# feifeibear/long-context-attention

Hardware: AMD Instinct MI355X
Metric: attention TFLOP/s (algorithmic, causal fwd+bwd) + iter ms of LongContextAttention at seqlen 64K, ulysses x ring (higher is better)
Workload: dtype bf16

## Files before the change

### long-context-attention_amd/csrc/usp_flash_bwd_dq64.hip

```cpp
#ifdef USP_Q64_TIMING
#define USP_TIMING
#endif
#include "usp_bwd_params.hpp"
#include "usp_host.hpp"
#include "usp_mfma64.hpp"

namespace usp {

#ifndef USP_Q64_PF
#define USP_Q64_PF 3
#endif
constexpr int kQ64_PF = USP_Q64_PF;
#ifndef USP_Q64_Y1
#define USP_Q64_Y1 24
#endif
constexpr int kQ64_Y1 = USP_Q64_Y1;

template <int DT, bool CAUSAL>
__global__ __launch_bounds__(256, 1) void flash_bwd_dq64_kernel(const BwdParams ) {
  using E = Elem<DT>;
  using M = M64<DT>;
  constexpr int D = 128, kBM = 256;
  constexpr int ROWB = D * 2;
  constexpr int TILEB = kTile * ROWB;
  constexpr int VOFF = 2 * TILEB;
  constexpr int NKT = D / 16, NDJ = D / 32;
  constexpr int PF = kQ64_PF;

  extern __shared__ __attribute__((aligned(16))) char smem_raw[];
  USP_LDS char* smem = lds_block_at_zero(smem_raw);

  const int tid = threadIdx.x;
  const int lane = tid & 63;
  const int wave = __builtin_amdgcn_readfirstlane(tid >> 6);
  const int l31 = lane & 31;
  const int hi = lane >> 5;
  typedef const __attribute__((address_space(4))) BwdParams* KArgs;
  KArgs p = (KArgs)__builtin_amdgcn_kernarg_segment_ptr();
  asm volatile("" : "+s"(p));

  const int dma_row = lane >> 4, dma_c8 = dma_lane_col(lane & 15, dma_row);
  const int k_voff = dma_row * (int)p->k_ss * 2 + dma_c8, v_voff = dma_row * (int)p->v_ss * 2 + dma_c8;
  const int rd_base = l31 * ROWB + ((hi ^ tile_swz<D>(l31)) * 16);
  int tr_addr[NDJ][2];
  {
    const int i = lane & 15, grp = (lane >> 4) & 1;
#pragma unroll
    for (int dj = 0; dj < NDJ; ++dj)
#pragma unroll
      for (int e = 0; e < 2; ++e) tr_addr[dj][e] = tr_read_offset<D>(i, grp, hi, dj, e);
  }
  const float c = p->scale_log2;

  const ItemWalk walk(p->n_items);
  for (int pass = 0;; ++pass) {
  int w = walk.at(pass);
  if (w < 0) break;
  asm volatile("" : "+s"(p));
  USP_TM(const uint64_t tm_item = __builtin_amdgcn_s_memtime();)
  w = walk.dealt(w, p->nblk);
  if (p->ksplit <= 1) w = walk.grouped(w, p->nblk, p->walk_g);
  const int qt_r = w % p->nblk;
  int rest = w / p->nblk;
  const int qt = CAUSAL ? (p->nblk - 1 - qt_r) : qt_r;
  int cut = 0;
  if (p->ksplit > 1) { cut = rest % p->ksplit; rest /= p->ksplit; }
  const int h = rest % p->Hq, b = rest / p->Hq;
  const int hkv = h / p->G;
  const int q0 = qt * kBM;
  const int qw = q0 + wave * 64;
  const int off = p->causal_off;

  const usp_query_tiles kr = usp_query_tiles_of(q0, kBM, qw, 64, p->Sq, p->Sk, CAUSAL, off, kTile);
  const int nt = kr.nt, n_w = kr.n_w, n_full = kr.n_full;
  usp_tile_run run = {0, nt};
  if (p->ksplit > 1) run = usp_equal_run(0, nt, p->ksplit, cut);
  const int tb = run.begin, te = run.end;
  const int e_full = usp_clamp_to_run(n_full, tb, te);
  const int e_own = usp_clamp_to_run(n_w, tb, te);

  u32x4 qf[2][NKT], df[2][NKT];
  float nl[2], dl[2];
#pragma unroll
  for (int qb = 0; qb < 2; ++qb) {
    const int row = qw + 32 * qb + l31;
    const int row_c = row < p->Sq ? row : p->Sq - 1;
    const char* qp = p->q + 2 * (b * p->q_sb + (int64_t)row_c * p->q_ss + h * p->q_sh) + 16 * hi;
    const char* dp = p->dout + 2 * (b * p->do_sb + (int64_t)row_c * p->do_ss + h * p->do_sh) + 16 * hi;
    load_resident16(qf[qb], df[qb], qp, dp);
    const float lse = p->lse[b * p->lse_sb + h * p->lse_sh + row_c];
    const float dlt = p->delta[b * p->dl_sb + h * p->dl_sh + row_c];
    const bool live = row < p->Sq && lse != USP_NEG_INF;
    nl[qb] = live ? -lse * kLog2e : USP_NEG_INF;
    dl[qb] = live ? dlt : 0.f;
  }

  const int k_rowb = (int)p->k_ss * 2, v_rowb = (int)p->v_ss * 2;
  const int64_t k_tb = (int64_t)kTile * k_rowb, v_tb = (int64_t)kTile * v_rowb;
  int k_step = 4 * k_rowb - 1024, v_step = 4 * v_rowb - 1024;
  int lds_w = wave * 4096;
  const char* k_cur = p->k + 2 * (b * p->k_sb + hkv * p->k_sh) + (int64_t)wave * 16 * k_rowb + tb * k_tb;
  const char* v_cur = p->v + 2 * (b * p->v_sb + hkv * p->v_sh) + (int64_t)wave * 16 * v_rowb + tb * v_tb;
  int rows_kv = p->Sk - 16 * wave - tb * kTile;
  u32x4 k_rs, v_rs;
  int dma_buf = 0;
  auto dma_open = [&](int buf) {
    k_rs = make_rsrc_rows(k_cur, rows_kv, 16, k_rowb, 2 * D);
    v_rs = make_rsrc_rows(v_cur, rows_kv, 16, v_rowb, 2 * D);
    dma_buf = buf;
    k_cur += k_tb;
    v_cur += v_tb;
    rows_kv -= kTile;
  };
  auto dma_piece = [&](int n) {
    asm volatile("" : "+s"(lds_w), "+s"(k_step), "+s"(v_step));
    const int i = n & 3;
    if (n < 4) lds_dma16_asm(k_rs, lds_w + dma_buf * TILEB, k_voff ^ (16 * i), i * k_step, i);
    else lds_dma16_asm(v_rs, lds_w + VOFF + dma_buf * TILEB, v_voff ^ (16 * i), i * v_step, i);
  };

  f32x16 dq[2][NDJ];
#pragma unroll
  for (int qb = 0; qb < 2; ++qb)
#pragma unroll
    for (int dj = 0; dj < NDJ; ++dj) zero_pin_agpr(dq[qb][dj]);

  dma_open(tb & 1);
#pragma unroll
  for (int n = 0; n < 8; ++n) dma_piece(n);
  dma_drain();
  __syncthreads();

  auto iter = [&](auto mask_c, int t, bool work) __attribute__((always_inline)) {
    constexpr bool MASK = decltype(mask_c)::value;
    const int par = t & 1;
    if (work) {
#pragma unroll
      for (int qb = 0; qb < 2; ++qb)
#pragma unroll
        for (int kt = 0; kt < NKT; ++kt) { pin_agpr4(qf[qb][kt]); pin_agpr4(df[qb][kt]); }
      int kr = rd_base + par * TILEB, vr = rd_base + VOFF + par * TILEB;
      asm volatile("" : "+v"(kr), "+v"(vr));
      USP_LDS const char* kt_base = smem + par * TILEB;
      f32x16 bs[2][2], bd[2][2];
      u32x4 pk[2][4];
      u32x4 ka[2 * NKT], va[2 * NKT], xa[4 * NDJ];
      auto rd_k = [&](int f) { ka[f] = *(USP_LDS const u32x4*)(smem + (f & 1) * 32 * ROWB + (kr ^ (32 * (f >> 1)))); };
      auto rd_v = [&](int f) { va[f] = *(USP_LDS const u32x4*)(smem + (f & 1) * 32 * ROWB + (vr ^ (32 * (f >> 1)))); };
      auto rd_x = [&](int f) {
        USP_LDS const char* xb = kt_base + (f / NDJ) * 16 * ROWB;
        const u32x2 a0 = lds_read_tr16(xb + tr_addr[f % NDJ][0]);
        const u32x2 a1 = lds_read_tr16(xb + tr_addr[f % NDJ][1]);
        xa[f] = u32x4{a0[0], a0[1], a1[0], a1[1]};
      };
      auto X = [&](int qb, int n) {
        const int ks = n >> 3, kb = ks >> 1, r = 8 * (ks & 1) + (n & 7);
        bs[qb][kb][r] = fast_exp2(__builtin_fmaf(bs[qb][kb][r], c, nl[qb]));
      };
      auto Y = [&](int qb, int n) {
        const int ks = n >> 3, kb = ks >> 1, r = 8 * (ks & 1) + (n & 7);
        bd[qb][kb][r] = (bd[qb][kb][r] - dl[qb]) * bs[qb][kb][r];
        if (r & 1) pk[qb][ks][(n & 7) >> 1] = E::pack2(bd[qb][kb][r - 1], bd[qb][kb][r]);
      };
      auto mask = [&](int qb) {
        const int row = qw + 32 * qb + l31;
        int klim = p->Sk - 1;
        if (CAUSAL) klim = row + off < klim ? row + off : klim;
        const int kb0 = t * kTile + 4 * hi;
#pragma unroll
        for (int r = 0; r < 16; ++r) {
          const int key = kb0 + (r & 3) + 8 * (r >> 2);
          if (key > klim) bs[qb][0][r] = USP_NEG_INF;
          if (key + 32 > klim) bs[qb][1][r] = USP_NEG_INF;
        }
      };
#pragma unroll
      for (int f = 0; f < PF; ++f) rd_k(f);
      __builtin_amdgcn_sched_barrier(0);
#pragma unroll
      for (int i = 0; i < 16; ++i) {
        const int kt = i >> 1, kb = i & 1;
        if (kt == 0) M::template s_first<MASK>(bs[0][kb], ka[i], qf[0][0]);
        else M::template s_next<MASK>(bs[0][kb], ka[i], qf[0][kt]);
        if (i == 0) { __builtin_amdgcn_sched_barrier(0); dma_open(par ^ 1); }
        if (i + PF < 16) rd_k(i + PF);
        if (i >= 1 && i <= 8) dma_piece(i - 1);
        __builtin_amdgcn_sched_barrier(0);
      }
      if (MASK) { mfma_settle(bs[0]); mask(0); }
#pragma unroll
      for (int i = 0; i < 16; ++i) {
        const int kt = i >> 1, kb = i & 1;
        if (kt == 0) M::template s_first<MASK>(bs[1][kb], ka[i], qf[1][0]);
        else M::template s_next<MASK>(bs[1][kb], ka[i], qf[1][kt]);
        if (i == 0) __builtin_amdgcn_sched_barrier(0);
        X(0, 2 * i); X(0, 2 * i + 1);
        if (i >= 16 - PF) rd_v(i - (16 - PF));
        __builtin_amdgcn_sched_barrier(0);
      }
      if (MASK) { mfma_settle(bs[1]); mask(1); }
#pragma unroll
      for (int i = 0; i < 16; ++i) {
        const int kt = i >> 1, kb = i & 1;
        if (kt == 0) M::template s_first<MASK>(bd[0][kb], va[i], df[0][0]);
        else M::template s_next<MASK>(bd[0][kb], va[i], df[0][kt]);
        if (i == 0) __builtin_amdgcn_sched_barrier(0);
        if (i + PF < 16) rd_v(i + PF);
        X(1, 2 * i); X(1, 2 * i + 1);
        __builtin_amdgcn_sched_barrier(0);
      }
#pragma unroll
      for (int i = 0; i < 16; ++i) {
        const int kt = i >> 1, kb = i & 1;
        if (kt == 0) M::template s_first<MASK>(bd[1][kb], va[i], df[1][0]);
        else M::template s_next<MASK>(bd[1][kb], va[i], df[1][kt]);
        if (i == 0) __builtin_amdgcn_sched_barrier(0);
        Y(0, 2 * i); Y(0, 2 * i + 1);
        if (i >= 16 - PF) rd_x(i - (16 - PF));
        __builtin_amdgcn_sched_barrier(0);
      }
      constexpr int NY1 = kQ64_Y1;
      static_assert(NY1 >= 16 && NY1 <= 28, "dS of k-step ks must be packed before gap 16 + 4 ks");
#pragma unroll
      for (int i = 0; i < 16; ++i) {
        M::template o_acc<MASK>(dq[0][i % NDJ], xa[i], pk[0][i / NDJ]);
        if (i == 0) __builtin_amdgcn_sched_barrier(0);
        if (i + PF < 16) rd_x(i + PF);
#pragma unroll
        for (int n = i * 32 / NY1; n < (i + 1) * 32 / NY1; ++n) Y(1, n);
        __builtin_amdgcn_sched_barrier(0);
      }
#pragma unroll
      for (int i = 0; i < 16; ++i) {
        M::template o_acc<MASK>(dq[1][i % NDJ], xa[i], pk[1][i / NDJ]);
        if (16 + i < NY1) {
#pragma unroll
          for (int n = (16 + i) * 32 / NY1; n < (16 + i + 1) * 32 / NY1; ++n) Y(1, n);
        }
        __builtin_amdgcn_sched_barrier(0);
      }
    } else {
      dma_open(par ^ 1);
#pragma unroll
      for (int n = 0; n < 8; ++n) dma_piece(n);
    }
    dma_drain();
    __syncthreads();
  };
  const std::integral_constant<bool, false> plain;
  const std::integral_constant<bool, true> masked;
  int t = tb;
  USP_TM(const uint64_t tm_loop = __builtin_amdgcn_s_memtime();)
  __builtin_amdgcn_s_waitcnt(0x0f70);
  for (; t < e_full; ++t) iter(plain, t, true);
  __builtin_amdgcn_s_waitcnt(0x0f70);
  for (; t < e_own; ++t) iter(masked, t, true);
  mfma_settle(dq);
  USP_TM(const uint64_t tm_own = __builtin_amdgcn_s_memtime(); const uint64_t tm_plain_n = n_full;)
  for (; t < te; ++t) iter(plain, t, false);
  USP_TM(const uint64_t tm_epi = __builtin_amdgcn_s_memtime();)

  mfma_settle(dq);
  asm volatile("" : "+s"(p));
  const bool wide = (p->wide16 & 1) != 0;
#pragma unroll
  for (int qb = 0; qb < 2; ++qb) {
    const int row = qw + 32 * qb + l31;
    if (wide) {
      const int row_c = row < p->Sq ? row : 0;
      store_row16_wide<E, NDJ>(p->dq16 + 2 * (b * p->dq16_sb + (int64_t)row_c * p->dq16_ss + h * p->dq16_sh), dq[qb], p->scale, hi,
                               row < p->Sq);
    } else if (row < p->Sq) {
      float* o1 = p->dq + b * p->dq_sb + (int64_t)row * p->dq_ss + h * p->dq_sh;
      char* h1 = p->dq16 ? p->dq16 + 2 * (b * p->dq16_sb + (int64_t)row * p->dq16_ss + h * p->dq16_sh) : nullptr;
      int acc_f = p->accum_dq;
      if (p->ksplit > 1) {
        o1 = p->ws_dq + ((((int64_t)cut * p->B + b) * p->Sq + row) * p->Hq + h) * D;
        h1 = nullptr;
        acc_f = 0;
      }
      store_row32_acc<E, NDJ>(o1, h1, dq[qb], p->scale, hi, acc_f);
    }
  }
  __syncthreads();
USP_TM(
  if (pass < 3 && lane == 0 && (blockIdx.x % 61) == 0)
    printf("TQ wg %3d pass %d wave %d qt %2d tiles own %3d (plain %3d) wg %3d : prologue %6llu own tiles %8llu (%5llu / tile) idle %6llu epilogue %6llu\n",
           (int)blockIdx.x, pass, wave, qt, n_w, (int)tm_plain_n, nt, (unsigned long long)(tm_loop - tm_item),
           (unsigned long long)(tm_own - tm_loop), (unsigned long long)((tm_own - tm_loop) / (n_w > 0 ? n_w : 1)),
           (unsigned long long)(tm_epi - tm_own), (unsigned long long)(__builtin_amdgcn_s_memtime() - tm_epi));
)
  }
}

bool dq64_serves(const BwdParams& p_in) {
  if (p_in.seq_q || p_in.seq_k || p_in.sched || p_in.win_on) return false;
  return dma_rows_ok(p_in.k_ss, true) && dma_rows_ok(p_in.v_ss, true);
}

bool launch_dq64(const BwdParams& p_in, int dtype, bool causal, hipStream_t st, int* rc) {
  if (!dq64_serves(p_in)) return false;
  BwdParams p = p_in;
  p.nblk = (p.Sq + 255) / 256;
  p.n_items = p.B * p.Hq * p.nblk * p.ksplit;
  p.wide16 = (p.ksplit <= 1 && p.dq16 && !p.accum_dq && tensor_aligned(p.dq16, p.dq16_sb, p.dq16_ss, p.dq16_sh, 16, 8)) ? 1 : 0;
  const int grid = persistent_grid(p.n_items, device_cus(), p.interleave);
  const size_t lds = 4 * kTile * 128 * 2;
  with_dtype_causal(dtype, causal, [&](auto dt, auto c) {
    hipLaunchKernelGGL((flash_bwd_dq64_kernel<decltype(dt)::value, decltype(c)::value>), dim3(grid), dim3(256), lds, st, p);
  });
  *rc = launched();
  return true;
}

}
```

Measured before the change: 986.8.

## Reorder dq64 backward chains by key block and share a rotating fragment ring

Restructures the dq-only backward iteration so the S and dP MFMA chains run per key block (kb) across both query blocks, instead of per query block. All K, V and transposed-K LDS fragments now go through a single 8-entry rotating register ring with grouped prefetch and explicit lgkmcnt waits. The delta subtraction is folded into the dP accumulator init via a new s_first_c with a pre-broadcast -delta vector, which removes one VALU op per element. This aims to cut register pressure and VALU work and to hide LDS latency better, at the cost of a tighter wait schedule, an extra 32 VGPRs for ndl, and reliance on a new M64 helper.

```diff
diff --git a/long-context-attention_amd/csrc/usp_flash_bwd_dq64.hip b/long-context-attention_amd/csrc/usp_flash_bwd_dq64.hip
--- a/long-context-attention_amd/csrc/usp_flash_bwd_dq64.hip
+++ b/long-context-attention_amd/csrc/usp_flash_bwd_dq64.hip
@@ -7,12 +7,8 @@
 
 namespace usp {
 
-#ifndef USP_Q64_PF
-#define USP_Q64_PF 3
-#endif
-constexpr int kQ64_PF = USP_Q64_PF;
 #ifndef USP_Q64_Y1
-#define USP_Q64_Y1 24
+#define USP_Q64_Y1 23
 #endif
 constexpr int kQ64_Y1 = USP_Q64_Y1;
 
@@ -25,7 +21,6 @@
   constexpr int TILEB = kTile * ROWB;
   constexpr int VOFF = 2 * TILEB;
   constexpr int NKT = D / 16, NDJ = D / 32;
-  constexpr int PF = kQ64_PF;
 
   extern __shared__ __attribute__((aligned(16))) char smem_raw[];
   USP_LDS char* smem = lds_block_at_zero(smem_raw);
@@ -80,7 +75,8 @@
   const int e_own = usp_clamp_to_run(n_w, tb, te);
 
   u32x4 qf[2][NKT], df[2][NKT];
-  float nl[2], dl[2];
+  float nl[2];
+  f32x16 ndl[2];
 #pragma unroll
   for (int qb = 0; qb < 2; ++qb) {
     const int row = qw + 32 * qb + l31;
@@ -92,7 +88,10 @@
     const float dlt = p->delta[b * p->dl_sb + h * p->dl_sh + row_c];
     const bool live = row < p->Sq && lse != USP_NEG_INF;
     nl[qb] = live ? -lse * kLog2e : USP_NEG_INF;
-    dl[qb] = live ? dlt : 0.f;
+    const float nd = live ? -dlt : 0.f;
+#pragma unroll
+    for (int r = 0; r < 16; ++r) ndl[qb][r] = nd;
+    asm volatile("" : "+v"(ndl[qb]));
   }
 
   const int k_rowb = (int)p->k_ss * 2, v_rowb = (int)p->v_ss * 2;
@@ -144,99 +143,103 @@
       USP_LDS const char* kt_base = smem + par * TILEB;
       f32x16 bs[2][2], bd[2][2];
       u32x4 pk[2][4];
-      u32x4 ka[2 * NKT], va[2 * NKT], xa[4 * NDJ];
-      auto rd_k = [&](int f) { ka[f] = *(USP_LDS const u32x4*)(smem + (f & 1) * 32 * ROWB + (kr ^ (32 * (f >> 1)))); };
-      auto rd_v = [&](int f) { va[f] = *(USP_LDS const u32x4*)(smem + (f & 1) * 32 * ROWB + (vr ^ (32 * (f >> 1)))); };
-      auto rd_x = [&](int f) {
-        USP_LDS const char* xb = kt_base + (f / NDJ) * 16 * ROWB;
-        const u32x2 a0 = lds_read_tr16(xb + tr_addr[f % NDJ][0]);
-        const u32x2 a1 = lds_read_tr16(xb + tr_addr[f % NDJ][1]);
-        xa[f] = u32x4{a0[0], a0[1], a1[0], a1[1]};
-      };
-      auto X = [&](int qb, int n) {
-        const int ks = n >> 3, kb = ks >> 1, r = 8 * (ks & 1) + (n & 7);
-        bs[qb][kb][r] = fast_exp2(__builtin_fmaf(bs[qb][kb][r], c, nl[qb]));
-      };
-      auto Y = [&](int qb, int n) {
-        const int ks = n >> 3, kb = ks >> 1, r = 8 * (ks & 1) + (n & 7);
-        bd[qb][kb][r] = (bd[qb][kb][r] - dl[qb]) * bs[qb][kb][r];
-        if (r & 1) pk[qb][ks][(n & 7) >> 1] = E::pack2(bd[qb][kb][r - 1], bd[qb][kb][r]);
-      };
-      auto mask = [&](int qb) {
-        const int row = qw + 32 * qb + l31;
-        int klim = p->Sk - 1;
-        if (CAUSAL) klim = row + off < klim ? row + off : klim;
-        const int kb0 = t * kTile + 4 * hi;
-#pragma unroll
-        for (int r = 0; r < 16; ++r) {
-          const int key = kb0 + (r & 3) + 8 * (r >> 2);
-          if (key > klim) bs[qb][0][r] = USP_NEG_INF;
-          if (key + 32 > klim) bs[qb][1][r] = USP_NEG_INF;
+      constexpr int NFR = 8;
+      u32x4 fr[NFR];
+      constexpr int NY1 = kQ64_Y1;
+      static_assert(NY1 >= 16 && NY1 <= 23, "dS of k-step 2 + k2 must be packed a gap before slot 80 + 8 k2 takes it");
+      auto rd = [&](int F, int e) {
+        u32x4& d = fr[F % NFR];
+        if (F < 32) {
+          const int b = F >> 3;
+          if (e == 0) d = *(USP_LDS const u32x4*)(smem + (b >> 1) * 32 * ROWB + ((b & 1 ? vr : kr) ^ (32 * (F & 7))));
+        } else {
+          const int f = F - 32;
+          const u32x2 h = lds_read_tr16(kt_base + (f / NDJ) * 16 * ROWB + tr_addr[f % NDJ][e]);
+          d[2 * e] = h[0];
+          d[2 * e + 1] = h[1];
         }
       };
-#pragma unroll
-      for (int f = 0; f < PF; ++f) rd_k(f);
+      auto rd_ahead = [&](int slot) {
+        const int F = 4 * ((slot >> 3) + 1) + (slot & 7);
+        if ((slot & 7) < 4 && F < 48) { rd(F, 0); rd(F, 1); }
+      };
+      auto group_wait = [&](int slot) {
+        if ((slot & 7) == 0) __builtin_amdgcn_s_waitcnt(0xc07f);
+      };
+      auto X = [&](int kb, int n) {
+        const int k2 = n >> 4, qb = (n >> 3) & 1, r = 8 * k2 + (n & 7);
+        bs[kb][qb][r] = fast_exp2(__builtin_fmaf(bs[kb][qb][r], c, nl[qb]));
+      };
+      auto Y = [&](int kb, int n) {
+        const int k2 = n >> 4, qb = (n >> 3) & 1, r = 8 * k2 + (n & 7);
+        bd[kb][qb][r] = bd[kb][qb][r] * bs[kb][qb][r];
+        if (r & 1) pk[qb][2 * kb + k2][(n & 7) >> 1] = E::pack2(bd[kb][qb][r - 1], bd[kb][qb][r]);
+      };
+      auto mask = [&](int kb) {
+        const int key0 = t * kTile + 32 * kb + 4 * hi;
+#pragma unroll
+        for (int qb = 0; qb < 2; ++qb) {
+          const int row = qw + 32 * qb + l31;
+          int klim = p->Sk - 1;
+          if (CAUSAL) klim = row + off < klim ? row + off : klim;
+#pragma unroll
+          for (int r = 0; r < 16; ++r)
+            if (key0 + (r & 3) + 8 * (r >> 2) > klim) bs[kb][qb][r] = USP_NEG_INF;
+        }
+      };
+      auto stream = [&](int g, int first, int span, auto&& fn) {
+        const int i = g - first;
+        if (i < 0 || i >= span) return;
+#pragma unroll
+        for (int n = i * 32 / span; n < (i + 1) * 32 / span; ++n) fn(n);
+      };
+      auto elems = [&](int g) {
+        stream(g, 16, 32, [&](int n) { X(0, n); });
+        stream(g, 32, 32, [&](int n) { Y(0, n); });
+        stream(g, 48, 32, [&](int n) { X(1, n); });
+        stream(g, 64, NY1, [&](int n) { Y(1, n); });
+      };
+      auto chain_block = [&](auto dp_c, int kb, int b) {
+        constexpr bool DP = decltype(dp_c)::value;
+#pragma unroll
+        for (int i = 0; i < 16; ++i) {
+          const int kt = i >> 1, qb = i & 1;
+          group_wait(16 * b + i);
+          const u32x4& a = fr[(8 * b + kt) % NFR];
+          f32x16& acc = DP ? bd[kb][qb] : bs[kb][qb];
+          const u32x4& bq = DP ? df[qb][kt] : qf[qb][kt];
+          if (kt == 0 && DP) M::template s_first_c<MASK>(acc, a, bq, ndl[qb]);
+          else if (kt == 0) M::template s_first<MASK>(acc, a, bq);
+          else M::template s_next<MASK>(acc, a, bq);
+          if (i == 0) {
+            __builtin_amdgcn_sched_barrier(0);
+            if (b == 0) dma_open(par ^ 1);
+          }
+          rd_ahead(16 * b + i);
+          if (b == 0 && i >= 1 && i <= 8) dma_piece(i - 1);
+          elems(16 * b + i);
+          __builtin_amdgcn_sched_barrier(0);
+        }
+      };
+      const std::integral_constant<bool, false> of_s;
+      const std::integral_constant<bool, true> of_dp;
+#pragma unroll
+      for (int F = 0; F < 4; ++F) { rd(F, 0); rd(F, 1); }
       __builtin_amdgcn_sched_barrier(0);
-#pragma unroll
-      for (int i = 0; i < 16; ++i) {
-        const int kt = i >> 1, kb = i & 1;
-        if (kt == 0) M::template s_first<MASK>(bs[0][kb], ka[i], qf[0][0]);
-        else M::template s_next<MASK>(bs[0][kb], ka[i], qf[0][kt]);
-        if (i == 0) { __builtin_amdgcn_sched_barrier(0); dma_open(par ^ 1); }
-        if (i + PF < 16) rd_k(i + PF);
-        if (i >= 1 && i <= 8) dma_piece(i - 1);
-        __builtin_amdgcn_sched_barrier(0);
-      }
+      chain_block(of_s, 0, 0);
       if (MASK) { mfma_settle(bs[0]); mask(0); }
-#pragma unroll
-      for (int i = 0; i < 16; ++i) {
-        const int kt = i >> 1, kb = i & 1;
-        if (kt == 0) M::template s_first<MASK>(bs[1][kb], ka[i], qf[1][0]);
-        else M::template s_next<MASK>(bs[1][kb], ka[i], qf[1][kt]);
+      chain_block(of_dp, 0, 1);
+      chain_block(of_s, 1, 2);
+      if (MASK) { mfma_settle(bs[1]); mask(1); }
+      chain_block(of_dp, 1, 3);
+#pragma unroll
+      for (int i = 0; i < 32; ++i) {
+        const int f = i >> 1, qb = i & 1;
+        group_wait(64 + i);
+        M::template o_acc<MASK>(dq[qb][f % NDJ], fr[(32 + f) % NFR], pk[qb][f / NDJ]);
         if (i == 0) __builtin_amdgcn_sched_barrier(0);
-        X(0, 2 * i); X(0, 2 * i + 1);
-        if (i >= 16 - PF) rd_v(i - (16 - PF));
-        __builtin_amdgcn_sched_barrier(0);
-      }
-      if (MASK) { mfma_settle(bs[1]); mask(1); }
-#pragma unroll
-      for (int i = 0; i < 16; ++i) {
-        const int kt = i >> 1, kb = i & 1;
-        if (kt == 0) M::template s_first<MASK>(bd[0][kb], va[i], df[0][0]);
-        else M::template s_next<MASK>(bd[0][kb], va[i], df[0][kt]);
-        if (i == 0) __builtin_amdgcn_sched_barrier(0);
-        if (i + PF < 16) rd_v(i + PF);
-        X(1, 2 * i); X(1, 2 * i + 1);
-        __builtin_amdgcn_sched_barrier(0);
-      }
-#pragma unroll
-      for (int i = 0; i < 16; ++i) {
-        const int kt = i >> 1, kb = i & 1;
-        if (kt == 0) M::template s_first<MASK>(bd[1][kb], va[i], df[1][0]);
-        else M::template s_next<MASK>(bd[1][kb], va[i], df[1][kt]);
-        if (i == 0) __builtin_amdgcn_sched_barrier(0);
-        Y(0, 2 * i); Y(0, 2 * i + 1);
-        if (i >= 16 - PF) rd_x(i - (16 - PF));
-        __builtin_amdgcn_sched_barrier(0);
-      }
-      constexpr int NY1 = kQ64_Y1;
-      static_assert(NY1 >= 16 && NY1 <= 28, "dS of k-step ks must be packed before gap 16 + 4 ks");
-#pragma unroll
-      for (int i = 0; i < 16; ++i) {
-        M::template o_acc<MASK>(dq[0][i % NDJ], xa[i], pk[0][i / NDJ]);
-        if (i == 0) __builtin_amdgcn_sched_barrier(0);
-        if (i + PF < 16) rd_x(i + PF);
-#pragma unroll
-        for (int n = i * 32 / NY1; n < (i + 1) * 32 / NY1; ++n) Y(1, n);
-        __builtin_amdgcn_sched_barrier(0);
-      }
-#pragma unroll
-      for (int i = 0; i < 16; ++i) {
-        M::template o_acc<MASK>(dq[1][i % NDJ], xa[i], pk[1][i / NDJ]);
-        if (16 + i < NY1) {
-#pragma unroll
-          for (int n = (16 + i) * 32 / NY1; n < (16 + i + 1) * 32 / NY1; ++n) Y(1, n);
-        }
+        rd_ahead(64 + i);
+        elems(64 + i);
         __builtin_amdgcn_sched_barrier(0);
       }
     } else {
```

New measurement: 992.9, median of 6. About the same (+0.6%).

## Reschedule dQ64 softmax/dS element streams and DMA pieces across MFMA gaps

Applied to the files above, without the earlier changes.

Replaces the fixed placement of the exp (X) and dS (Y) elementwise work and of the K/V DMA pieces with configurable constexpr streams spread over all 96 MFMA gaps. The streams are checked at compile time against the dependency rules. The -dl subtraction moves into the dP MFMA accumulator init through s_first_c with a precomputed cd vector, which saves one VALU op per element. It also adds optional per-block timing stamps, which are compiled only under USP_TIMING, and it uses extra VGPRs for cd.

```diff
diff --git a/long-context-attention_amd/csrc/usp_flash_bwd_dq64.hip b/long-context-attention_amd/csrc/usp_flash_bwd_dq64.hip
--- a/long-context-attention_amd/csrc/usp_flash_bwd_dq64.hip
+++ b/long-context-attention_amd/csrc/usp_flash_bwd_dq64.hip
@@ -7,14 +7,62 @@
 
 namespace usp {
 
+#ifdef USP_TIMING
+USP_DEV uint32_t tm_stamp() {
+  __builtin_amdgcn_sched_barrier(0);
+  const uint32_t t = (uint32_t)__builtin_amdgcn_s_memtime();
+  __builtin_amdgcn_sched_barrier(0);
+  return t;
+}
+#endif
+
 #ifndef USP_Q64_PF
 #define USP_Q64_PF 3
 #endif
 constexpr int kQ64_PF = USP_Q64_PF;
-#ifndef USP_Q64_Y1
-#define USP_Q64_Y1 24
-#endif
-constexpr int kQ64_Y1 = USP_Q64_Y1;
+#ifndef USP_Q64_DMA_OPEN
+#define USP_Q64_DMA_OPEN -1
+#endif
+#ifndef USP_Q64_DMA_P0
+#define USP_Q64_DMA_P0 1
+#endif
+#ifndef USP_Q64_DMA_PS
+#define USP_Q64_DMA_PS 2
+#endif
+#ifndef USP_Q64_XB2
+#define USP_Q64_XB2 28
+#endif
+#ifndef USP_Q64_XB4
+#define USP_Q64_XB4 20
+#endif
+#ifndef USP_Q64_YB4
+#define USP_Q64_YB4 16
+#endif
+constexpr int kQ64_XB2 = USP_Q64_XB2, kQ64_XB4 = USP_Q64_XB4, kQ64_XB3 = 64 - kQ64_XB2 - kQ64_XB4, kQ64_YB4 = USP_Q64_YB4;
+static_assert(kQ64_XB2 >= 1 && kQ64_XB3 >= 1 && kQ64_XB4 >= 0 && kQ64_YB4 >= 1 && kQ64_YB4 <= 32 && kQ64_YB4 % 2 == 0, "element streams");
+constexpr int q64_gap_x(int e) {
+  if (e < kQ64_XB2) return 16 + e * 16 / kQ64_XB2;
+  if (e < kQ64_XB2 + kQ64_XB3) return 32 + (e - kQ64_XB2) * 16 / kQ64_XB3;
+  return 48 + (e - kQ64_XB2 - kQ64_XB3) * 16 / (kQ64_XB4 > 0 ? kQ64_XB4 : 1);
+}
+constexpr int q64_gap_y(int e) {
+  if (e < kQ64_YB4) return 48 + e * 16 / kQ64_YB4;
+  return 64 + (e - kQ64_YB4) / 2;
+}
+constexpr bool q64_streams_ok() {
+  for (int e = 0; e < 64; ++e) {
+    const int qb = e >> 5, ks = (e & 31) >> 3;
+    if (q64_gap_x(e) < 16 + 16 * qb) return false;
+    if (q64_gap_y(e) < 48 + 16 * qb || q64_gap_y(e) < q64_gap_x(e)) return false;
+    if (q64_gap_y(e) >= 64 + 16 * qb + 4 * ks) return false;
+    if (e && (q64_gap_x(e) < q64_gap_x(e - 1) || q64_gap_y(e) < q64_gap_y(e - 1))) return false;
+  }
+  return true;
+}
+static_assert(q64_streams_ok(), "dS of k-step ks must be packed before gap 16 + 4 ks of its dQ block, from complete chains");
+constexpr int kQ64_DmaOpen = USP_Q64_DMA_OPEN, kQ64_DmaP0 = USP_Q64_DMA_P0, kQ64_DmaPS = USP_Q64_DMA_PS;
+static_assert(kQ64_DmaOpen >= -1 && kQ64_DmaOpen < kQ64_DmaP0 && kQ64_DmaPS >= 1, "the descriptors are made before the first piece");
+static_assert(kQ64_DmaP0 + 7 * kQ64_DmaPS < 80, "every piece is issued a block (16 gaps) or more before the dma_drain");
 
 template <int DT, bool CAUSAL>
 __global__ __launch_bounds__(256, 1) void flash_bwd_dq64_kernel(const BwdParams ) {
@@ -119,6 +167,14 @@
     else lds_dma16_asm(v_rs, lds_w + VOFF + dma_buf * TILEB, v_voff ^ (16 * i), i * v_step, i);
   };
 
+  f32x16 cd[2];
+#pragma unroll
+  for (int qb = 0; qb < 2; ++qb) {
+#pragma unroll
+    for (int r = 0; r < 16; ++r) cd[qb][r] = -dl[qb];
+    asm volatile("" : "+v"(cd[qb]));
+  }
+
   f32x16 dq[2][NDJ];
 #pragma unroll
   for (int qb = 0; qb < 2; ++qb)
@@ -131,10 +187,13 @@
   dma_drain();
   __syncthreads();
 
+  USP_TM(uint32_t tm_blk[8] = {0, 0, 0, 0, 0, 0, 0, 0};)
   auto iter = [&](auto mask_c, int t, bool work) __attribute__((always_inline)) {
     constexpr bool MASK = decltype(mask_c)::value;
     const int par = t & 1;
+    USP_TM(uint32_t tm_s[8] = {0, 0, 0, 0, 0, 0, 0, 0};)
     if (work) {
+      USP_TM(tm_s[0] = tm_stamp();)
 #pragma unroll
       for (int qb = 0; qb < 2; ++qb)
 #pragma unroll
@@ -159,8 +218,22 @@
       };
       auto Y = [&](int qb, int n) {
         const int ks = n >> 3, kb = ks >> 1, r = 8 * (ks & 1) + (n & 7);
-        bd[qb][kb][r] = (bd[qb][kb][r] - dl[qb]) * bs[qb][kb][r];
+        bd[qb][kb][r] = bd[qb][kb][r] * bs[qb][kb][r];
         if (r & 1) pk[qb][ks][(n & 7) >> 1] = E::pack2(bd[qb][kb][r - 1], bd[qb][kb][r]);
+      };
+      auto elems = [&](int g) {
+#pragma unroll
+        for (int e = 0; e < 64; ++e)
+          if (q64_gap_x(e) == g) X(e >> 5, e & 31);
+#pragma unroll
+        for (int e = 0; e < 64; ++e)
+          if (q64_gap_y(e) == g) Y(e >> 5, e & 31);
+      };
+      auto stage = [&](int g) {
+        if (g == kQ64_DmaOpen) dma_open(par ^ 1);
+#pragma unroll
+        for (int n = 0; n < 8; ++n)
+          if (g == kQ64_DmaP0 + n * kQ64_DmaPS) dma_piece(n);
       };
       auto mask = [&](int qb) {
         const int row = qw + 32 * qb + l31;
@@ -176,17 +249,19 @@
       };
 #pragma unroll
       for (int f = 0; f < PF; ++f) rd_k(f);
+      if (kQ64_DmaOpen < 0) dma_open(par ^ 1);
       __builtin_amdgcn_sched_barrier(0);
 #pragma unroll
       for (int i = 0; i < 16; ++i) {
         const int kt = i >> 1, kb = i & 1;
         if (kt == 0) M::template s_first<MASK>(bs[0][kb], ka[i], qf[0][0]);
         else M::template s_next<MASK>(bs[0][kb], ka[i], qf[0][kt]);
-        if (i == 0) { __builtin_amdgcn_sched_barrier(0); dma_open(par ^ 1); }
+        if (i == 0) __builtin_amdgcn_sched_barrier(0);
         if (i + PF < 16) rd_k(i + PF);
-        if (i >= 1 && i <= 8) dma_piece(i - 1);
-        __builtin_amdgcn_sched_barrier(0);
-      }
+        stage(i);
+        __builtin_amdgcn_sched_barrier(0);
+      }
+      USP_TM(tm_s[1] = tm_stamp();)
       if (MASK) { mfma_settle(bs[0]); mask(0); }
 #pragma unroll
       for (int i = 0; i < 16; ++i) {
@@ -194,51 +269,54 @@
         if (kt == 0) M::template s_first<MASK>(bs[1][kb], ka[i], qf[1][0]);
         else M::template s_next<MASK>(bs[1][kb], ka[i], qf[1][kt]);
         if (i == 0) __builtin_amdgcn_sched_barrier(0);
-        X(0, 2 * i); X(0, 2 * i + 1);
+        elems(16 + i);
         if (i >= 16 - PF) rd_v(i - (16 - PF));
-        __builtin_amdgcn_sched_barrier(0);
-      }
+        stage(16 + i);
+        __builtin_amdgcn_sched_barrier(0);
+      }
+      USP_TM(tm_s[2] = tm_stamp();)
       if (MASK) { mfma_settle(bs[1]); mask(1); }
 #pragma unroll
       for (int i = 0; i < 16; ++i) {
         const int kt = i >> 1, kb = i & 1;
-        if (kt == 0) M::template s_first<MASK>(bd[0][kb], va[i], df[0][0]);
+        if (kt == 0) M::template s_first_c<MASK>(bd[0][kb], va[i], df[0][0], cd[0]);
         else M::template s_next<MASK>(bd[0][kb], va[i], df[0][kt]);
         if (i == 0) __builtin_amdgcn_sched_barrier(0);
         if (i + PF < 16) rd_v(i + PF);
-        X(1, 2 * i); X(1, 2 * i + 1);
-        __builtin_amdgcn_sched_barrier(0);
-      }
+        elems(32 + i);
+        stage(32 + i);
+        __builtin_amdgcn_sched_barrier(0);
+      }
+      USP_TM(tm_s[3] = tm_stamp();)
 #pragma unroll
       for (int i = 0; i < 16; ++i) {
         const int kt = i >> 1, kb = i & 1;
-        if (kt == 0) M::template s_first<MASK>(bd[1][kb], va[i], df[1][0]);
+        if (kt == 0) M::template s_first_c<MASK>(bd[1][kb], va[i], df[1][0], cd[1]);
         else M::template s_next<MASK>(bd[1][kb], va[i], df[1][kt]);
         if (i == 0) __builtin_amdgcn_sched_barrier(0);
-        Y(0, 2 * i); Y(0, 2 * i + 1);
+        elems(48 + i);
         if (i >= 16 - PF) rd_x(i - (16 - PF));
-        __builtin_amdgcn_sched_barrier(0);
-      }
-      constexpr int NY1 = kQ64_Y1;
-      static_assert(NY1 >= 16 && NY1 <= 28, "dS of k-step ks must be packed before gap 16 + 4 ks");
+        stage(48 + i);
+        __builtin_amdgcn_sched_barrier(0);
+      }
+      USP_TM(tm_s[4] = tm_stamp();)
 #pragma unroll
       for (int i = 0; i < 16; ++i) {
         M::template o_acc<MASK>(dq[0][i % NDJ], xa[i], pk[0][i / NDJ]);
         if (i == 0) __builtin_amdgcn_sched_barrier(0);
         if (i + PF < 16) rd_x(i + PF);
-#pragma unroll
-        for (int n = i * 32 / NY1; n < (i + 1) * 32 / NY1; ++n) Y(1, n);
-        __builtin_amdgcn_sched_barrier(0);
-      }
+        elems(64 + i);
+        stage(64 + i);
+        __builtin_amdgcn_sched_barrier(0);
+      }
+      USP_TM(tm_s[5] = tm_stamp();)
 #pragma unroll
       for (int i = 0; i < 16; ++i) {
         M::template o_acc<MASK>(dq[1][i % NDJ], xa[i], pk[1][i / NDJ]);
-        if (16 + i < NY1) {
-#pragma unroll
-          for (int n = (16 + i) * 32 / NY1; n < (16 + i + 1) * 32 / NY1; ++n) Y(1, n);
-        }
-        __builtin_amdgcn_sched_barrier(0);
-      }
+        elems(80 + i);
+        __builtin_amdgcn_sched_barrier(0);
+      }
+      USP_TM(tm_s[6] = tm_stamp();)
     } else {
       dma_open(par ^ 1);
 #pragma unroll
@@ -246,6 +324,11 @@
     }
     dma_drain();
     __syncthreads();
+    USP_TM(if (work && !MASK) {
+      tm_s[7] = tm_stamp();
+      _Pragma("unroll") for (int j = 0; j < 7; ++j) tm_blk[j] += tm_s[j + 1] - tm_s[j];
+      ++tm_blk[7];
+    })
   };
   const std::integral_constant<bool, false> plain;
   const std::integral_constant<bool, true> masked;
@@ -284,11 +367,13 @@
   }
   __syncthreads();
 USP_TM(
+  const uint32_t tm_n = tm_blk[7] ? tm_blk[7] : 1;
   if (pass < 3 && lane == 0 && (blockIdx.x % 61) == 0)
-    printf("TQ wg %3d pass %d wave %d qt %2d tiles own %3d (plain %3d) wg %3d : prologue %6llu own tiles %8llu (%5llu / tile) idle %6llu epilogue %6llu\n",
+    printf("TQ wg %3d pass %d wave %d qt %2d tiles own %3d (plain %3d) wg %3d : prologue %6llu own tiles %8llu (%5llu / tile) idle %6llu epilogue %6llu | plain tile B1-B6, drain + barrier: %u %u %u %u %u %u %u\n",
            (int)blockIdx.x, pass, wave, qt, n_w, (int)tm_plain_n, nt, (unsigned long long)(tm_loop - tm_item),
            (unsigned long long)(tm_own - tm_loop), (unsigned long long)((tm_own - tm_loop) / (n_w > 0 ? n_w : 1)),
-           (unsigned long long)(tm_epi - tm_own), (unsigned long long)(__builtin_amdgcn_s_memtime() - tm_epi));
+           (unsigned long long)(tm_epi - tm_own), (unsigned long long)(__builtin_amdgcn_s_memtime() - tm_epi),
+           tm_blk[0] / tm_n, tm_blk[1] / tm_n, tm_blk[2] / tm_n, tm_blk[3] / tm_n, tm_blk[4] / tm_n, tm_blk[5] / tm_n, tm_blk[6] / tm_n);
 )
   }
 }
```

New measurement: 1039 before, 1051 after (median of 6 runs). 1.2% higher.
